# ikt-luh/Unified-Point-Cloud-Compression

Hardware: AMD Instinct MI355X
Metric: points/sec encode+decode, longdress vox10, 1 GPU; bpp & D1-PSNR parity (higher is better)
Workload: dtype f32

## Files before the change

unified_point_cloud_compression_amd/csrc/pcc_conv_thin.hip:

```cpp
#include "pcc_conv.h"

struct ThinArgs {
  const float* feat; const float* wt; const float* bias;
  const int* hdr; const int* nbr; const int* rows;
  float* out; long long n_out; int cin, cout, act; float slope; int lpr_log2;
};

template <int COUT_MAX, int VEC>
__global__ void __launch_bounds__(256) k_conv_thin(ThinArgs a) {
  typedef typename ThinVec<VEC>::T VT;
  constexpr int JB = 9;
  const int lane = threadIdx.x & 63;
  const int lpr = 1 << a.lpr_log2;
  const int rpw = 64 >> a.lpr_log2;
  const long long wave = (long long)blockIdx.x * 4 + (threadIdx.x >> 6);
  const long long p = wave * rpw + (lane >> a.lpr_log2);
  const int cl = lane & (lpr - 1);
  const bool valid = p < a.n_out;
  const int cvec = a.cin / VEC;

  int k_count = 1, koff_begin = 0;
  long long seg_pos_count = a.n_out, local = p;
  const int* seg_nbr = nullptr;
  const bool identity = (a.hdr == nullptr);
  if (!identity && valid) {
    const int nseg = a.hdr[HDR_NSEG];
    int s = 0;
    for (; s < nseg - 1; ++s) {
      const int* sg = a.hdr + HDR_SEG0 + s * SEG_WORDS;
      if (p < (long long)sg[SEG_POS_BEGIN] + sg[SEG_POS_COUNT]) break;
    }
    const int* sg = a.hdr + HDR_SEG0 + s * SEG_WORDS;
    k_count = sg[SEG_K_COUNT];
    koff_begin = sg[SEG_KOFF_BEGIN];
    seg_pos_count = sg[SEG_POS_COUNT];
    local = p - sg[SEG_POS_BEGIN];
    seg_nbr = a.nbr + (((long long)(unsigned)sg[SEG_NBR_LO]) | ((long long)sg[SEG_NBR_HI] << 32));
  }
  float acc[COUT_MAX];
#pragma unroll
  for (int o = 0; o < COUT_MAX; ++o) acc[o] = 0.f;
  if (valid) {
    for (int cv = cl; cv < cvec; cv += lpr) {
      for (int j0 = 0; j0 < k_count; j0 += JB) {
        int ir[JB];
#pragma unroll
        for (int u = 0; u < JB; ++u) {
          const int j = j0 + u;
          ir[u] = (j < k_count) ? (identity ? (int)p : seg_nbr[(long long)j * seg_pos_count + local]) : -1;
        }
        VT x[JB];
#pragma unroll
        for (int u = 0; u < JB; ++u) {
          thin_zero(x[u]);
          if (ir[u] >= 0) x[u] = reinterpret_cast<const VT*>(a.feat + (long long)ir[u] * a.cin)[cv];
        }
#pragma unroll
        for (int u = 0; u < JB; ++u) {
          const int j = j0 + u;
          if (j < k_count) {
            const int kid = identity ? 0 : a.hdr[HDR_KOFFS + koff_begin + j];
            const float* wk = a.wt + (long long)kid * a.cout * a.cin;
#pragma unroll
            for (int o = 0; o < COUT_MAX; ++o)
              if (o < a.cout) acc[o] += thin_dot(x[u], reinterpret_cast<const VT*>(wk + o * a.cin)[cv]);
          }
        }
      }
    }
  }
#pragma unroll
  for (int o = 0; o < COUT_MAX; ++o)
    for (int d = lpr >> 1; d >= 1; d >>= 1) acc[o] += __shfl_xor(acc[o], d);
  if (valid && cl == 0) {
    const long long orow = a.rows ? a.rows[p] : p;
#pragma unroll
    for (int o = 0; o < COUT_MAX; ++o) {
      if (o >= a.cout) break;
      float v = acc[o] + (a.bias ? a.bias[o] : 0.f);
      if (a.act == PCC_ACT_RELU) v = fmaxf(v, 0.f);
      else if (a.act == PCC_ACT_LEAKY) v = v >= 0.f ? v : v * a.slope;
      a.out[orow * a.cout + o] = v;
    }
  }
}

template <int CIN>
__global__ void __launch_bounds__(256) k_thin_project(const float* __restrict__ feat, long long n_in,
                                                      const float* __restrict__ wt, int kc, float* __restrict__ t) {
  extern __shared__ __attribute__((aligned(16))) float w_s[];
  for (int i = threadIdx.x; i < kc * CIN; i += 256) w_s[i] = wt[i];
  __syncthreads();
  const long long i = (long long)blockIdx.x * 256 + threadIdx.x;
  if (i >= n_in) return;
  float4 x[CIN / 4];
#pragma unroll
  for (int c = 0; c < CIN / 4; ++c) x[c] = reinterpret_cast<const float4*>(feat + i * CIN)[c];
  for (int k = 0; k < kc; ++k) {
    float acc = 0.f;
#pragma unroll
    for (int c = 0; c < CIN / 4; ++c) {
      const float4 w = reinterpret_cast<const float4*>(w_s + k * CIN)[c];
      acc += x[c].x * w.x + x[c].y * w.y + x[c].z * w.z + x[c].w * w.w;
    }
    t[(long long)k * n_in + i] = acc;
  }
}

struct ThinGatherArgs {
  const float* t; const float* bias; const int* hdr; const int* nbr; const int* rows;
  float* out; long long n_in, n_out; int cout, act; float slope;
};

template <int COUT_MAX>
__global__ void __launch_bounds__(256) k_thin_gather(ThinGatherArgs a) {
  constexpr int JB = 9;
  const long long p = (long long)blockIdx.x * 256 + threadIdx.x;
  if (p >= a.n_out) return;
  int k_count = 1, koff_begin = 0;
  long long spc = a.n_out, local = p;
  const int* seg_nbr = nullptr;
  const bool identity = (a.hdr == nullptr);
  if (!identity) {
    const int nseg = a.hdr[HDR_NSEG];
    int s = 0;
    for (; s < nseg - 1; ++s) {
      const int* sg = a.hdr + HDR_SEG0 + s * SEG_WORDS;
      if (p < (long long)sg[SEG_POS_BEGIN] + sg[SEG_POS_COUNT]) break;
    }
    const int* sg = a.hdr + HDR_SEG0 + s * SEG_WORDS;
    k_count = sg[SEG_K_COUNT]; koff_begin = sg[SEG_KOFF_BEGIN]; spc = sg[SEG_POS_COUNT];
    local = p - sg[SEG_POS_BEGIN];
    seg_nbr = a.nbr + (((long long)(unsigned)sg[SEG_NBR_LO]) | ((long long)sg[SEG_NBR_HI] << 32));
  }
  float acc[COUT_MAX];
#pragma unroll
  for (int o = 0; o < COUT_MAX; ++o) acc[o] = 0.f;
  for (int j0 = 0; j0 < k_count; j0 += JB) {
    int ir[JB];
#pragma unroll
    for (int u = 0; u < JB; ++u)
      ir[u] = (j0 + u < k_count) ? (identity ? (int)p : seg_nbr[(long long)(j0 + u) * spc + local]) : -1;
    float v[JB][COUT_MAX];
#pragma unroll
    for (int u = 0; u < JB; ++u) {
      const int kid = (ir[u] >= 0 && !identity) ? a.hdr[HDR_KOFFS + koff_begin + j0 + u] : 0;
#pragma unroll
      for (int o = 0; o < COUT_MAX; ++o)
        v[u][o] = (ir[u] >= 0 && o < a.cout) ? a.t[(long long)(kid * a.cout + o) * a.n_in + ir[u]] : 0.f;
    }
#pragma unroll
    for (int u = 0; u < JB; ++u)
#pragma unroll
      for (int o = 0; o < COUT_MAX; ++o) acc[o] += v[u][o];
  }
  const long long orow = a.rows ? a.rows[p] : p;
#pragma unroll
  for (int o = 0; o < COUT_MAX; ++o)
    if (o < a.cout) a.out[orow * a.cout + o] = act1(acc[o] + (a.bias ? a.bias[o] : 0.f), a.act, a.slope);
}


struct Wave16Args {
  const float* feat; const float* wl; const float* bias; const int* hdr; const int* nbr; const int* rows;
  float* out; long long n_out, n_in; int K, cout, act; float slope;
  const int* tiles = nullptr; const int* n_tiles = nullptr;
  const float* w2 = nullptr;
  float* t = nullptr;
};

template <int CIN>
__device__ __forceinline__ const float* wave16_w(const float* wl_s, int kid, int kq, int r16) {
  return wl_s + ((kid * (CIN / 4) + kq) * 16 + r16) * 4;
}

template <int CIN>
__global__ void __launch_bounds__(512) k_conv_wave16(Wave16Args a) {
  constexpr int G = CIN / 16;
  constexpr int NW = 8;
  extern __shared__ __attribute__((aligned(16))) float wl_s[];
  for (int i = threadIdx.x; i < a.K * 16 * (CIN / 4); i += 512)
    reinterpret_cast<float4*>(wl_s)[i] = reinterpret_cast<const float4*>(a.wl)[i];
  __syncthreads();
  const int lane = threadIdx.x & 63, r16 = lane & 15, q = lane >> 4;
  const bool identity = (a.hdr == nullptr);
  const int nseg = identity ? 1 : a.hdr[HDR_NSEG];
  long long total_tiles = 0;
  if (identity) total_tiles = (a.n_out + 31) / 32;
  else
    for (int s = 0; s < nseg; ++s) total_tiles += (a.hdr[HDR_SEG0 + s * SEG_WORDS + SEG_POS_COUNT] + 31) / 32;

  const int cpx = gridDim.x >> 3;
  const long long per_xcd = (total_tiles + 7) / 8;
  const long long xcd_lo = (long long)(blockIdx.x & 7) * per_xcd;
  const long long xcd_hi = min(total_tiles, xcd_lo + per_xcd);
  for (long long wt = xcd_lo + (long long)(blockIdx.x >> 3) * NW + (threadIdx.x >> 6); wt < xcd_hi;
       wt += (long long)cpx * NW) {
    long long pos0, spc;
    int npos, k_count = 1, koff_begin = 0;
    const int* seg_nbr = nullptr;
    if (identity) {
      pos0 = wt * 32; npos = (int)min(32ll, a.n_out - pos0); spc = a.n_out;
    } else {
      long long tile = wt;
      int s = 0;
      for (; s < nseg - 1; ++s) {
        const long long tiles = (a.hdr[HDR_SEG0 + s * SEG_WORDS + SEG_POS_COUNT] + 31) / 32;
        if (tile < tiles) break;
        tile -= tiles;
      }
      const int* sg = a.hdr + HDR_SEG0 + s * SEG_WORDS;
      k_count = sg[SEG_K_COUNT]; koff_begin = sg[SEG_KOFF_BEGIN]; spc = sg[SEG_POS_COUNT];
      const long long local0 = tile * 32;
      pos0 = sg[SEG_POS_BEGIN] + local0;
      npos = (int)min(32ll, spc - local0);
      seg_nbr = a.nbr + (((long long)(unsigned)sg[SEG_NBR_LO]) | ((long long)sg[SEG_NBR_HI] << 32)) + local0;
    }
    const bool vA = r16 < npos, vB = 16 + r16 < npos;
    f32x4 accA0 = {0.f, 0.f, 0.f, 0.f}, accA1 = accA0, accB0 = accA0, accB1 = accA0;
    auto fetch = [&](int j, int& iA, int& iB) {
      iA = -1; iB = -1;
      if (j < k_count) {
        if (vA) iA = identity ? (int)(pos0 + r16) : seg_nbr[(long long)j * spc + r16];
        if (vB) iB = identity ? (int)(pos0 + 16 + r16) : seg_nbr[(long long)j * spc + 16 + r16];
      }
    };
    auto gather = [&](int iA, int iB, float4 (&xa)[G], float4 (&xb)[G]) {
#pragma unroll
      for (int g = 0; g < G; ++g) {
        xa[g] = make_float4(0.f, 0.f, 0.f, 0.f);
        xb[g] = xa[g];
        if (iA >= 0) xa[g] = *reinterpret_cast<const float4*>(a.feat + (long long)iA * CIN + 16 * g + 4 * q);
        if (iB >= 0) xb[g] = *reinterpret_cast<const float4*>(a.feat + (long long)iB * CIN + 16 * g + 4 * q);
      }
    };
    int iA0, iB0, iA1, iB1, iA2, iB2;
    float4 xa[G], xb[G], ya[G], yb[G];
    fetch(0, iA0, iB0);
    fetch(1, iA1, iB1);
    gather(iA0, iB0, xa, xb);
    for (int j = 0; j < k_count; ++j) {
      fetch(j + 2, iA2, iB2);
      gather(iA1, iB1, ya, yb);
      if (__ballot(iA0 >= 0 || iB0 >= 0)) {
        const int kid = identity ? 0 : a.hdr[HDR_KOFFS + koff_begin + j];
#pragma unroll
        for (int g = 0; g < G; ++g) {
          const float4 w = *reinterpret_cast<const float4*>(wave16_w<CIN>(wl_s, kid, 4 * g + q, r16));
          accA0 = __builtin_amdgcn_mfma_f32_16x16x4f32(xa[g].x, w.x, accA0, 0, 0, 0);
          accB0 = __builtin_amdgcn_mfma_f32_16x16x4f32(xb[g].x, w.x, accB0, 0, 0, 0);
          accA1 = __builtin_amdgcn_mfma_f32_16x16x4f32(xa[g].y, w.y, accA1, 0, 0, 0);
          accB1 = __builtin_amdgcn_mfma_f32_16x16x4f32(xb[g].y, w.y, accB1, 0, 0, 0);
          accA0 = __builtin_amdgcn_mfma_f32_16x16x4f32(xa[g].z, w.z, accA0, 0, 0, 0);
          accB0 = __builtin_amdgcn_mfma_f32_16x16x4f32(xb[g].z, w.z, accB0, 0, 0, 0);
          accA1 = __builtin_amdgcn_mfma_f32_16x16x4f32(xa[g].w, w.w, accA1, 0, 0, 0);
          accB1 = __builtin_amdgcn_mfma_f32_16x16x4f32(xb[g].w, w.w, accB1, 0, 0, 0);
        }
      }
#pragma unroll
      for (int g = 0; g < G; ++g) { xa[g] = ya[g]; xb[g] = yb[g]; }
      iA0 = iA1; iB0 = iB1; iA1 = iA2; iB1 = iB2;
    }
    if (r16 < a.cout) {
      const float b = a.bias ? a.bias[r16] : 0.f;
#pragma unroll
      for (int e = 0; e < 4; ++e) {
        const int rA = 4 * q + e, rB = 16 + 4 * q + e;
        if (rA < npos) {
          const long long orow = a.rows ? a.rows[pos0 + rA] : pos0 + rA;
          a.out[orow * a.cout + r16] = act1(accA0[e] + accA1[e] + b, a.act, a.slope);
        }
        if (rB < npos) {
          const long long orow = a.rows ? a.rows[pos0 + rB] : pos0 + rB;
          a.out[orow * a.cout + r16] = act1(accB0[e] + accB1[e] + b, a.act, a.slope);
        }
      }
    }
  }
}

template <int CTRL>
__device__ __forceinline__ int dpp_i(int v) { return __builtin_amdgcn_update_dpp(0, v, CTRL, 0xF, 0xF, true); }
template <int CTRL>
__device__ __forceinline__ float dpp_f(float v) {
  return __builtin_bit_cast(float, __builtin_amdgcn_update_dpp(0, __builtin_bit_cast(int, v), CTRL, 0xF, 0xF, true));
}
static constexpr int DPP_SHL1 = 0x101, DPP_SHR1 = 0x111;

template <int CIN, bool PROJ>
__global__ void __launch_bounds__(512) k_conv_wave16z(Wave16Args a) {
  constexpr int G = CIN / 16;
  constexpr int NW = 8;
  extern __shared__ __attribute__((aligned(16))) float wl_s[];
  for (int i = threadIdx.x; i < 27 * 16 * (CIN / 4); i += 512)
    reinterpret_cast<float4*>(wl_s)[i] = reinterpret_cast<const float4*>(a.wl)[i];
  __syncthreads();
  const int lane = threadIdx.x & 63, r16 = lane & 15, q = lane >> 4;
  const unsigned spc = (unsigned)a.n_out;
  const unsigned total_tiles = a.tiles ? (unsigned)*a.n_tiles : (spc + 15) / 16;
  const unsigned cpx = gridDim.x >> 3;
  const unsigned per_xcd = (total_tiles + 7) / 8;
  const unsigned xcd_lo = (blockIdx.x & 7) * per_xcd;
  const unsigned xcd_hi = min(total_tiles, xcd_lo + per_xcd);
  const float* wl_lane = wl_s + r16 * 4 + q * 64;

  float w2r[2][4];
  float* hs = nullptr;
  if constexpr (PROJ) {
#pragma unroll
    for (int nt = 0; nt < 2; ++nt)
#pragma unroll
      for (int j = 0; j < 4; ++j) {
        const int k = 16 * nt + r16, c = 4 * j + q;
        w2r[nt][j] = (k < 27 && c < a.cout) ? a.w2[k * a.cout + c] : 0.f;
      }
    hs = wl_s + 27 * 16 * CIN + (threadIdx.x >> 6) * (16 * 17);
  }

  struct Grp { float4 c[G], m[G], p[G]; unsigned km, kp; };
  const __amdgpu_buffer_rsrc_t rs = __builtin_amdgcn_make_buffer_rsrc(
      const_cast<float*>(a.feat), (short)0, (int)(unsigned)((size_t)a.n_in * CIN * 4), 0x00020000);
  constexpr unsigned OOB = 0xFFFFFF00u;

  for (unsigned wt = xcd_lo + (blockIdx.x >> 3) * NW + (threadIdx.x >> 6); wt < xcd_hi; wt += cpx * NW) {
    unsigned pos0, npos;
    if (a.tiles) {
      const unsigned tw = (unsigned)a.tiles[wt];
      pos0 = tw & 0x07FFFFFFu; npos = (tw >> 27) + 1;
    } else {
      pos0 = wt * 16; npos = min(16u, spc - pos0);
    }
    const unsigned r = pos0 + min((unsigned)r16, npos - 1);
    const int* nb = a.nbr + r;
    f32x4 acc0 = {0.f, 0.f, 0.f, 0.f}, acc1 = acc0, acc2 = acc0, acc3 = acc0;

    auto issue = [&](int im, int ic, int ip, Grp& x) {
      const int cm = dpp_i<DPP_SHR1>(ic), cp = dpp_i<DPP_SHL1>(ic);
      const bool mm = im >= 0 && im == cm && r16 != 0;
      const bool mp = ip >= 0 && ip == cp && r16 != 15;
      x.km = mm ? 0xFFFFFFFFu : 0u;
      x.kp = mp ? 0xFFFFFFFFu : 0u;
      asm volatile("" : "+v"(x.km), "+v"(x.kp));
      const unsigned oc = ic >= 0 ? (unsigned)ic * (CIN * 4) + 16 * q : OOB;
      const unsigned om = (im >= 0 && !mm) ? (unsigned)im * (CIN * 4) + 16 * q : OOB;
      const unsigned op = (ip >= 0 && !mp) ? (unsigned)ip * (CIN * 4) + 16 * q : OOB;
#pragma unroll
      for (int g = 0; g < G; ++g) {
        x.c[g] = __builtin_bit_cast(float4, __builtin_amdgcn_raw_buffer_load_b128(rs, oc + 64 * g, 0, 0));
        x.m[g] = __builtin_bit_cast(float4, __builtin_amdgcn_raw_buffer_load_b128(rs, om + 64 * g, 0, 0));
        x.p[g] = __builtin_bit_cast(float4, __builtin_amdgcn_raw_buffer_load_b128(rs, op + 64 * g, 0, 0));
      }
    };
    auto mfma4 = [&](const float4& x, int slot, int g) {
      const float4 w = *reinterpret_cast<const float4*>(wl_lane + (slot * (CIN / 4) + 4 * g) * 64);
      acc0 = __builtin_amdgcn_mfma_f32_16x16x4f32(x.x, w.x, acc0, 0, 0, 0);
      acc1 = __builtin_amdgcn_mfma_f32_16x16x4f32(x.y, w.y, acc1, 0, 0, 0);
      acc2 = __builtin_amdgcn_mfma_f32_16x16x4f32(x.z, w.z, acc2, 0, 0, 0);
      acc3 = __builtin_amdgcn_mfma_f32_16x16x4f32(x.w, w.w, acc3, 0, 0, 0);
    };
    auto mix = [](unsigned k, float shifted, float loaded) {
      return __builtin_bit_cast(float, (__builtin_bit_cast(unsigned, shifted) & k) | __builtin_bit_cast(unsigned, loaded));
    };

    int im1 = nb[spc], ic1 = nb[10ull * spc], ip1 = nb[19ull * spc];
    Grp x, y;
    issue(nb[0], nb[9ull * spc], nb[18ull * spc], x);
    auto compute = [&](const Grp& x, int g9) {
#pragma unroll
      for (int g = 0; g < G; ++g) {
        float4 vm, vp;
        vm.x = mix(x.km, dpp_f<DPP_SHR1>(x.c[g].x), x.m[g].x);  vp.x = mix(x.kp, dpp_f<DPP_SHL1>(x.c[g].x), x.p[g].x);
        vm.y = mix(x.km, dpp_f<DPP_SHR1>(x.c[g].y), x.m[g].y);  vp.y = mix(x.kp, dpp_f<DPP_SHL1>(x.c[g].y), x.p[g].y);
        vm.z = mix(x.km, dpp_f<DPP_SHR1>(x.c[g].z), x.m[g].z);  vp.z = mix(x.kp, dpp_f<DPP_SHL1>(x.c[g].z), x.p[g].z);
        vm.w = mix(x.km, dpp_f<DPP_SHR1>(x.c[g].w), x.m[g].w);  vp.w = mix(x.kp, dpp_f<DPP_SHL1>(x.c[g].w), x.p[g].w);
        mfma4(vm, g9, g);
        mfma4(x.c[g], g9 + 9, g);
        mfma4(vp, g9 + 18, g);
      }
    };
#pragma unroll 1
    for (int g9 = 0; g9 < 8; g9 += 2) {
      const unsigned ga = (unsigned)(g9 + 2), gb = (unsigned)min(g9 + 3, 8);
      const int am = nb[(size_t)ga * spc], ac = nb[(size_t)(ga + 9) * spc], ap = nb[(size_t)(ga + 18) * spc];
      issue(im1, ic1, ip1, y);
      __builtin_amdgcn_sched_barrier(0);
      compute(x, g9);
      __builtin_amdgcn_sched_barrier(0);
      const int bm = nb[(size_t)gb * spc], bc = nb[(size_t)(gb + 9) * spc], bp = nb[(size_t)(gb + 18) * spc];
      issue(am, ac, ap, x);
      __builtin_amdgcn_sched_barrier(0);
      compute(y, g9 + 1);
      __builtin_amdgcn_sched_barrier(0);
      im1 = bm; ic1 = bc; ip1 = bp;
    }
    compute(x, 8);
    const float b = (a.bias && r16 < a.cout) ? a.bias[r16] : 0.f;
    if constexpr (!PROJ) {
      if (r16 < a.cout) {
#pragma unroll
        for (int e = 0; e < 4; ++e) {
          const unsigned lr = 4 * q + e;
          if (lr < npos) a.out[(size_t)(pos0 + lr) * a.cout + r16] = act1(acc0[e] + acc1[e] + acc2[e] + acc3[e] + b, a.act, a.slope);
        }
      }
    } else {
#pragma unroll
      for (int e = 0; e < 4; ++e)
        hs[(4 * q + e) * 17 + r16] = r16 < a.cout ? act1(acc0[e] + acc1[e] + acc2[e] + acc3[e] + b, a.act, a.slope) : 0.f;
      __builtin_amdgcn_wave_barrier();
      f32x4 d0 = {0.f, 0.f, 0.f, 0.f}, d1 = d0;
#pragma unroll
      for (int j = 0; j < 4; ++j) {
        const float hv = hs[r16 * 17 + 4 * j + q];
        d0 = __builtin_amdgcn_mfma_f32_16x16x4f32(w2r[0][j], hv, d0, 0, 0, 0);
        d1 = __builtin_amdgcn_mfma_f32_16x16x4f32(w2r[1][j], hv, d1, 0, 0, 0);
      }
      __builtin_amdgcn_wave_barrier();
      if ((unsigned)r16 < npos) {
        float* tp = a.t + (size_t)(4 * q) * spc + pos0 + r16;
#pragma unroll
        for (int e = 0; e < 4; ++e) {
          tp[(size_t)e * spc] = d0[e];
          if (16 + 4 * q + e < 27) tp[(size_t)(16 + e) * spc] = d1[e];
        }
      }
    }
  }
}

static bool g_wave16_zrun = getenv("PCC_WAVE16_ZRUN") ? atoi(getenv("PCC_WAVE16_ZRUN")) != 0 : true;

template <int CIN>
static int launch_wave16(const Wave16Args& a, hipStream_t s) {
  const size_t lds = (size_t)a.K * 16 * CIN * sizeof(float);
  int dev = 0;
  PCC_CHECK_HIP(hipGetDevice(&dev));
  static unsigned long long attr_set = 0;
  if (!(attr_set >> (dev & 63) & 1ull)) {
    PCC_CHECK_HIP(hipFuncSetAttribute((const void*)k_conv_wave16<CIN>, hipFuncAttributeMaxDynamicSharedMemorySize, 64 * 1024));
    PCC_CHECK_HIP(hipFuncSetAttribute((const void*)k_conv_wave16z<CIN, false>, hipFuncAttributeMaxDynamicSharedMemorySize, 64 * 1024));
    PCC_CHECK_HIP(hipFuncSetAttribute((const void*)k_conv_wave16z<CIN, true>, hipFuncAttributeMaxDynamicSharedMemorySize, 64 * 1024));
    attr_set |= 1ull << (dev & 63);
  }
  prof_note(PCC_FORM_WAVE16, 0.0, 0.0);
  prof_tile(32, 16, 1);
  const long long tiles = pcc_cdiv(a.n_out, 32) + (a.rows ? PCC_MAP_MAX_SEG : 0);
  long long want = pcc_cdiv(tiles, 8);
  want = (want + 7) / 8 * 8;
  const unsigned grid = (unsigned)(want < 512 ? want : 512);
  if (g_wave16_zrun && a.K == 27 && a.hdr && !a.rows && a.n_out * 27 < (1ll << 31) &&
      a.n_in * CIN * 4 <= 0xFFFFFE00ll) {
    if (a.t) k_conv_wave16z<CIN, true><<<grid, 512, lds + 8 * 16 * 17 * sizeof(float), s>>>(a);
    else k_conv_wave16z<CIN, false><<<grid, 512, lds, s>>>(a);
    PCC_LAUNCH_CHECK();
    return PCC_OK;
  }
  PCC_REQUIRE(!a.t, "pcc_conv_head_fwd: the fused head needs a canonical 3x3x3 map (one segment, no row list)");
  k_conv_wave16<CIN><<<grid, 512, lds, s>>>(a);
  PCC_LAUNCH_CHECK();
  return PCC_OK;
}

template <int CIN>
__global__ void __launch_bounds__(256) k_thin_project_mfma(const float* __restrict__ feat, long long n_in,
                                                           const float* __restrict__ wt, int kc, float* __restrict__ t) {
  constexpr int HC = CIN / 2, NV = HC / 4;
  const int lane = threadIdx.x & 63, r31 = lane & 31, half = lane >> 5;
  const long long ntiles = (n_in + 31) / 32;
  float wa[HC];
#pragma unroll
  for (int c = 0; c < HC; ++c) wa[c] = r31 < kc ? wt[r31 * CIN + half * HC + c] : 0.f;
  const long long tstep = (long long)gridDim.x * 4;
  long long tile = (long long)blockIdx.x * 4 + (threadIdx.x >> 6);
  if (tile >= ntiles) return;
  auto load = [&](long long tl, float4 (&x)[NV]) {
    long long row = tl * 32 + r31;
    if (row >= n_in) row = n_in - 1;
    const float4* src = reinterpret_cast<const float4*>(feat + row * CIN + half * HC);
#pragma unroll
    for (int v = 0; v < NV; ++v) x[v] = src[v];
  };
  auto run = [&](long long tl, const float4 (&x)[NV]) {
    f32x16 acc;
#pragma unroll
    for (int e = 0; e < 16; ++e) acc[e] = 0.f;
#pragma unroll
    for (int v = 0; v < NV; ++v) {
      acc = __builtin_amdgcn_mfma_f32_32x32x2f32(wa[4 * v + 0], x[v].x, acc, 0, 0, 0);
      acc = __builtin_amdgcn_mfma_f32_32x32x2f32(wa[4 * v + 1], x[v].y, acc, 0, 0, 0);
      acc = __builtin_amdgcn_mfma_f32_32x32x2f32(wa[4 * v + 2], x[v].z, acc, 0, 0, 0);
      acc = __builtin_amdgcn_mfma_f32_32x32x2f32(wa[4 * v + 3], x[v].w, acc, 0, 0, 0);
    }
    const long long row = tl * 32 + r31;
    if (row < n_in) {
#pragma unroll
      for (int e = 0; e < 16; ++e) {
        const int k = cfrag_row(0, e, half);
        if (k < kc) t[(long long)k * n_in + row] = acc[e];
      }
    }
  };
  float4 xa[NV], xb[NV];
  load(tile, xa);
  for (;;) {
    const long long t1 = tile + tstep;
    if (t1 < ntiles) load(t1, xb);
    run(tile, xa);
    if (t1 >= ntiles) break;
    const long long t2 = t1 + tstep;
    if (t2 < ntiles) load(t2, xa);
    run(t1, xb);
    if (t2 >= ntiles) break;
    tile = t2;
  }
}

template <int CIN>
static int launch_project(const float* feat, int64_t n_in, const float* wt, int kc, float* t, hipStream_t s) {
  if constexpr (CIN >= 32) {
    if (kc <= 32) {
      const long long tiles = pcc_cdiv(n_in, 32);
      long long grid = pcc_cdiv(tiles, 4 * 4);
      if (grid > 4096) grid = 4096;
      if (grid < 1) grid = 1;
      k_thin_project_mfma<CIN><<<(unsigned)grid, 256, 0, s>>>(feat, n_in, wt, kc, t);
      PCC_LAUNCH_CHECK();
      return PCC_OK;
    }
  }
  k_thin_project<CIN><<<(unsigned)pcc_cdiv(n_in, 256), 256, (size_t)kc * CIN * sizeof(float), s>>>(feat, n_in, wt, kc, t);
  PCC_LAUNCH_CHECK();
  return PCC_OK;
}

int launch_conv_wave16(const float* feat_in, int64_t n_in, int32_t cin, const float* packed_w, const float* bias, int32_t K,
                       int32_t cout, const int32_t* hdr, const int32_t* nbr, const int32_t* rows, int64_t n_out, float* out,
                       int32_t act, float slope, hipStream_t s, const int32_t* tiles, const int32_t* n_tiles, const float* w2,
                       float* t) {
  Wave16Args a;
  a.feat = feat_in; a.wl = packed_w; a.bias = bias; a.hdr = hdr; a.nbr = nbr; a.rows = rows; a.out = out;
  a.n_out = n_out; a.n_in = n_in; a.K = K; a.cout = cout; a.act = act; a.slope = slope;
  a.tiles = tiles; a.n_tiles = n_tiles; a.w2 = w2; a.t = t;
  if (cin == 16) PCC_TRY(launch_wave16<16>(a, s));
  else if (cin == 32) PCC_TRY(launch_wave16<32>(a, s));
  else PCC_TRY(launch_wave16<64>(a, s));
  return PCC_OK;
}

int launch_conv_thin_t(const float* feat_in, int64_t n_in, int32_t cin, const float* packed_w, const float* bias, int32_t K,
                       int32_t cout, const int32_t* hdr, const int32_t* nbr, const int32_t* rows, int64_t n_out, float* out,
                       int32_t act, float slope, void* ws, size_t ws_bytes, hipStream_t s) {
  if (!ws || ws_bytes < pcc_conv_ws_bytes(n_in, K, cin, cout)) {
    pcc_set_error("pcc_conv_fwd: workspace too small (need pcc_conv_ws_bytes)");
    return PCC_EWS;
  }
  float* t = (float*)ws;
  const int kc = K * cout;
  switch (cin) {
    case 4: PCC_TRY(launch_project<4>(feat_in, n_in, packed_w, kc, t, s)); break;
    case 8: PCC_TRY(launch_project<8>(feat_in, n_in, packed_w, kc, t, s)); break;
    case 16: PCC_TRY(launch_project<16>(feat_in, n_in, packed_w, kc, t, s)); break;
    case 32: PCC_TRY(launch_project<32>(feat_in, n_in, packed_w, kc, t, s)); break;
    default: PCC_TRY(launch_project<64>(feat_in, n_in, packed_w, kc, t, s)); break;
  }
  ThinGatherArgs g;
  g.t = t; g.bias = bias; g.hdr = hdr; g.nbr = nbr; g.rows = rows; g.out = out; g.n_in = n_in; g.n_out = n_out;
  g.cout = cout; g.act = act; g.slope = slope;
  k_thin_gather<4><<<(unsigned)pcc_cdiv(n_out, 256), 256, 0, s>>>(g);
  PCC_LAUNCH_CHECK();
  return PCC_OK;
}

int launch_conv_thin(const float* feat_in, int32_t cin, const float* packed_w, const float* bias, int32_t cout, const int32_t* hdr,
                     const int32_t* nbr, const int32_t* rows, int64_t n_out, float* out, int32_t act, float slope, hipStream_t s) {
  ThinArgs t;
  t.feat = feat_in; t.wt = packed_w; t.bias = bias; t.hdr = hdr; t.nbr = nbr; t.rows = rows; t.out = out;
  t.n_out = n_out; t.cin = cin; t.cout = cout; t.act = act; t.slope = slope;
  const int vec = (cin % 4 == 0) ? 4 : 1;
  int l = 0;
  while ((1 << l) < cin / vec && l < 6) ++l;
  t.lpr_log2 = l;
  const int64_t rpw = 64 >> l;
  const int64_t waves = pcc_cdiv(n_out, rpw);
  if (vec == 4) k_conv_thin<4, 4><<<(unsigned)pcc_cdiv(waves, 4), 256, 0, s>>>(t);
  else k_conv_thin<4, 1><<<(unsigned)pcc_cdiv(waves, 4), 256, 0, s>>>(t);
  PCC_LAUNCH_CHECK();
  return PCC_OK;
}

__global__ void k_band_segments(const long long* __restrict__ keys, long long n, int lo_x, int nx, int lo_y, int ny, int ts,
                                int nbands, int band_h, int* __restrict__ seg_row0, int* __restrict__ seg_tiles) {
  const int sidx = blockIdx.x * blockDim.x + threadIdx.x;
  if (sidx >= nbands * nx) return;
  const int band = sidx / nx, xi = sidx - band * nx;
  const long long x = (long long)lo_x + (long long)xi * ts + PCC_BIAS;
  const int cy0 = band * band_h, cy1 = min(ny, cy0 + band_h);
  auto lower = [&](long long key) {
    long long lo = 0, hi = n;
    while (lo < hi) {
      const long long mid = (lo + hi) >> 1;
      if (keys[mid] < key) lo = mid + 1; else hi = mid;
    }
    return lo;
  };
  long long b = 0, e = 0;
  if (cy0 < cy1) {
    const long long y0 = (long long)lo_y + (long long)cy0 * ts + PCC_BIAS, y1 = (long long)lo_y + (long long)cy1 * ts + PCC_BIAS;
    b = lower((x << PCC_KEY_X_SHIFT) | (y0 << PCC_KEY_Y_SHIFT));
    e = lower((x << PCC_KEY_X_SHIFT) | (y1 << PCC_KEY_Y_SHIFT));
  }
  seg_row0[sidx] = (int)b;
  seg_tiles[sidx] = (int)((e - b + 15) / 16);
  seg_row0[nbands * nx + sidx] = (int)(e - b);
}

__global__ void __launch_bounds__(1024) k_band_scan(const int* __restrict__ seg_tiles, int nseg, int* __restrict__ seg_tile0,
                                                    int* __restrict__ n_tiles) {
  __shared__ int part[1024];
  const int per = (nseg + 1023) / 1024;
  const int b = threadIdx.x * per, e = min(nseg, b + per);
  int sum = 0;
  for (int i = b; i < e; ++i) sum += seg_tiles[i];
  part[threadIdx.x] = sum;
  __syncthreads();
  for (int d = 1; d < 1024; d <<= 1) {
    const int v = threadIdx.x >= d ? part[threadIdx.x - d] : 0;
    __syncthreads();
    part[threadIdx.x] += v;
    __syncthreads();
  }
  int run = part[threadIdx.x] - sum;
  for (int i = b; i < e; ++i) { seg_tile0[i] = run; run += seg_tiles[i]; }
  if (threadIdx.x == 1023) *n_tiles = part[1023];
}

__global__ void __launch_bounds__(256) k_band_fill(const int* __restrict__ seg_row0, const int* __restrict__ seg_rows,
                                                   const int* __restrict__ seg_tile0, int nseg, int* __restrict__ tiles) {
  const int sidx = blockIdx.x * 4 + (threadIdx.x >> 6);
  if (sidx >= nseg) return;
  const int rows = seg_rows[sidx], r0 = seg_row0[sidx], t0 = seg_tile0[sidx];
  const int nt = (rows + 15) / 16;
  for (int j = threadIdx.x & 63; j < nt; j += 64) {
    const int cnt = min(16, rows - 16 * j);
    tiles[t0 + j] = (r0 + 16 * j) | ((cnt - 1) << 27);
  }
}

extern "C" int64_t pcc_band_tiles_cap(int64_t n, int32_t nx, int32_t nbands) { return n / 16 + (int64_t)nx * nbands + 16; }
extern "C" size_t pcc_band_tiles_ws_bytes(int32_t nx, int32_t nbands) { return pcc_align_up((size_t)nx * nbands * 4) * 4 + 256; }

extern "C" int pcc_band_tiles_build(const int64_t* keys, int64_t n, int32_t lo_x, int32_t nx, int32_t lo_y, int32_t ny,
                                    int32_t ts, int32_t nbands, int32_t* tiles, int64_t tiles_cap, int32_t* n_tiles,
                                    void* ws, size_t ws_bytes, void* stream) {
  hipStream_t s = (hipStream_t)stream;
  PCC_REQUIRE(keys && tiles && n_tiles && ws && n > 0 && n < (1ll << 27), "pcc_band_tiles_build: bad arguments (rows must stay below 2^27)");
  PCC_REQUIRE(nx >= 1 && ny >= 1 && ts >= 1 && nbands >= 1 && (int64_t)nx * nbands <= (1 << 20), "pcc_band_tiles_build: bad lattice");
  PCC_REQUIRE(tiles_cap >= pcc_band_tiles_cap(n, nx, nbands), "pcc_band_tiles_build: tile table too small (pcc_band_tiles_cap)");
  if (ws_bytes < pcc_band_tiles_ws_bytes(nx, nbands)) { pcc_set_error("pcc_band_tiles_build: workspace too small"); return PCC_EWS; }
  const int nseg = nx * nbands;
  const size_t st = pcc_align_up((size_t)nseg * 4);
  int* seg_row0 = (int*)ws;
  int* seg_tiles = (int*)((char*)ws + 2 * st);
  int* seg_tile0 = (int*)((char*)ws + 3 * st);
  PCC_REQUIRE(st >= (size_t)nseg * 4, "pcc_band_tiles_build: internal");
  const int band_h = (ny + nbands - 1) / nbands;
  k_band_segments<<<(unsigned)pcc_cdiv(nseg, 256), 256, 0, s>>>((const long long*)keys, n, lo_x, nx, lo_y, ny, ts, nbands, band_h,
                                                                seg_row0, seg_tiles);
  PCC_LAUNCH_CHECK();
  k_band_scan<<<1, 1024, 0, s>>>(seg_tiles, nseg, seg_tile0, n_tiles);
  PCC_LAUNCH_CHECK();
  k_band_fill<<<(unsigned)pcc_cdiv(nseg, 4), 256, 0, s>>>(seg_row0, seg_row0 + nseg, seg_tile0, nseg, tiles);
  PCC_LAUNCH_CHECK();
  return PCC_OK;
}

extern "C" int pcc_conv_head_supported(int32_t cin, int32_t cmid) {
  return (cmid > 4 && cmid <= 16 && conv_kind(27, cin, cmid) == KIND_WAVE16 && (size_t)27 * 16 * cin * 4 + 8 * 16 * 17 * 4 <= 64 * 1024) ? 1 : 0;
}
extern "C" size_t pcc_conv_head_ws_bytes(int64_t n) { return (size_t)27 * (size_t)(n > 0 ? n : 1) * sizeof(float) + 256; }

extern "C" int pcc_conv_head_fwd(const float* feat, int64_t n, int32_t cin, const float* packed_w0, const float* bias0,
                                 int32_t cmid, const float* w2, const float* bias2, const int32_t* hdr, const int32_t* nbr,
                                 const int32_t* tiles, const int32_t* n_tiles, float* logits, void* ws, size_t ws_bytes,
                                 void* stream) {
  hipStream_t s = (hipStream_t)stream;
  if (n <= 0) return PCC_OK;
  PCC_REQUIRE(feat && packed_w0 && w2 && hdr && nbr && logits && ws, "pcc_conv_head_fwd: NULL array");
  PCC_REQUIRE(pcc_conv_head_supported(cin, cmid), "pcc_conv_head_fwd: unsupported shape cin=%d cmid=%d", cin, cmid);
  PCC_REQUIRE((tiles == nullptr) == (n_tiles == nullptr), "pcc_conv_head_fwd: tiles and n_tiles go together");
  PCC_REQUIRE(n * 27 < (1ll << 31) && n * cin * 4 <= 0xFFFFFE00ll && g_wave16_zrun, "pcc_conv_head_fwd: set too large for 32-bit offsets");
  if (ws_bytes < pcc_conv_head_ws_bytes(n)) { pcc_set_error("pcc_conv_head_fwd: workspace too small"); return PCC_EWS; }
  PCC_TRY(prof_begin(s));
  PCC_TRY(launch_conv_wave16(feat, n, cin, packed_w0, bias0, 27, cmid, hdr, nbr, nullptr, n, nullptr, PCC_ACT_RELU, 0.f, s, tiles,
                             n_tiles, w2, (float*)ws));
  PCC_TRY(prof_end(s));
  ThinGatherArgs g;
  g.t = (const float*)ws; g.bias = bias2; g.hdr = hdr; g.nbr = nbr; g.rows = nullptr; g.out = logits; g.n_in = n; g.n_out = n;
  g.cout = 1; g.act = PCC_ACT_NONE; g.slope = 0.f;
  k_thin_gather<1><<<(unsigned)pcc_cdiv(n, 256), 256, 0, s>>>(g);
  PCC_LAUNCH_CHECK();
  return PCC_OK;
}

struct ThinGridArgs {
  const float* t; const float* bias; const long long* keys; PccGrid g; float* out; long long n; int cout;
};

template <int COUT_MAX>
__global__ void __launch_bounds__(256) k_thin_gather_grid(ThinGridArgs a) {
  const long long p = (long long)blockIdx.x * 256 + threadIdx.x;
  if (p >= a.n) return;
  const PccGrid& g = a.g;
  const long long key = a.keys[p];
  const PccLattice& L = g.lat;
  const int b = pcc_key_b(key);
  const int cx = (pcc_key_x(key) - L.lo[0]) >> L.ts_log2;
  const int cy = (pcc_key_y(key) - L.lo[1]) >> L.ts_log2;
  const int cz = (pcc_key_z(key) - L.lo[2]) >> L.ts_log2;
  const int z_lo = cz > 0 ? cz - 1 : 0, z_hi = cz + 1 < L.dims[2] ? cz + 1 : L.dims[2] - 1;
  const int nz = z_hi - z_lo + 1;
  float acc[COUT_MAX];
#pragma unroll
  for (int o = 0; o < COUT_MAX; ++o) acc[o] = 0.f;
#pragma unroll
  for (int c = 0; c < 9; ++c) {
    const int nx = cx + c % 3 - 1, ny = cy + c / 3 - 1;
    if (nx < 0 || ny < 0 || nx >= L.dims[0] || ny >= L.dims[1]) continue;
    const long long cell = (((long long)b * L.dims[0] + nx) * L.dims[1] + ny) * L.dims[2] + z_lo;
    const long long wi = cell >> 6;
    const int sh = (int)(cell & 63);
    const unsigned long long w0 = g.bits[wi];
    unsigned long long f64 = w0 >> sh;
    if (sh + nz > 64) f64 |= g.bits[wi + 1] << (64 - sh);
    unsigned f = (unsigned)f64 & ((1u << nz) - 1u);
    if (!f) continue;
    int r = g.rank[wi] + __popcll(w0 & ((1ull << sh) - 1ull));
    while (f) {
      const int t = __ffs((int)f) - 1;
      f &= f - 1;
      const int k = c + 9 * (z_lo + t - cz + 1);
#pragma unroll
      for (int o = 0; o < COUT_MAX; ++o)
        if (o < a.cout) acc[o] += a.t[(long long)(k * a.cout + o) * a.n + r];
      ++r;
    }
  }
#pragma unroll
  for (int o = 0; o < COUT_MAX; ++o)
    if (o < a.cout) a.out[p * a.cout + o] = acc[o] + (a.bias ? a.bias[o] : 0.f);
}

__global__ void __launch_bounds__(256) k_thin_gather_grid1(ThinGridArgs a) {
  const long long p = (long long)blockIdx.x * 256 + threadIdx.x;
  if (p >= a.n) return;
  const PccGrid& g = a.g;
  const long long key = a.keys[p];
  const PccLattice& L = g.lat;
  const int b = pcc_key_b(key);
  const int cx = (pcc_key_x(key) - L.lo[0]) >> L.ts_log2;
  const int cy = (pcc_key_y(key) - L.lo[1]) >> L.ts_log2;
  const int cz = (pcc_key_z(key) - L.lo[2]) >> L.ts_log2;
  const int z_lo = cz > 0 ? cz - 1 : 0, z_hi = cz + 1 < L.dims[2] ? cz + 1 : L.dims[2] - 1;
  const int nz = z_hi - z_lo + 1;
  const int dz0 = z_lo - cz + 1;
  unsigned long long w0[9], w1[9];
  int rk[9], sh[9];
  bool ok[9];
#pragma unroll
  for (int c = 0; c < 9; ++c) {
    const int nx = cx + c % 3 - 1, ny = cy + c / 3 - 1;
    ok[c] = !(nx < 0 || ny < 0 || nx >= L.dims[0] || ny >= L.dims[1]);
    const long long cell = ok[c] ? pcc_lat_cell(L, b, nx, ny, z_lo) : 0ll;
    const long long wi = cell >> 6;
    sh[c] = (int)(cell & 63);
    w0[c] = g.bits[wi];
    rk[c] = g.rank[wi];
    w1[c] = (sh[c] + nz > 64) ? g.bits[wi + 1] : 0ull;
  }
  const __amdgpu_buffer_rsrc_t rsT = __builtin_amdgcn_make_buffer_rsrc(const_cast<float*>(a.t), (short)0,
                                                                       (int)(unsigned)((size_t)27 * a.n * 4), 0x00020000);
  float v[27];
#pragma unroll
  for (int c = 0; c < 9; ++c) {
    unsigned long long f64 = w0[c] >> sh[c];
    if (sh[c] + nz > 64) f64 |= w1[c] << (64 - sh[c]);
    const unsigned f = ok[c] ? ((unsigned)f64 & ((1u << nz) - 1u)) : 0u;
    const int r = rk[c] + __popcll(w0[c] & ((1ull << sh[c]) - 1ull));
#pragma unroll
    for (int t = 0; t < 3; ++t) {
      const int k = c + 9 * (dz0 + t);
      const unsigned row = (unsigned)(r + __popc(f & ((1u << t) - 1u)));
      const unsigned off = ((f >> t) & 1u) ? ((unsigned)k * (unsigned)a.n + row) * 4u : BUF_OOB;
      v[c * 3 + t] = __builtin_bit_cast(float, __builtin_amdgcn_raw_buffer_load_b32(rsT, off, 0, 0));
    }
  }
  float acc = 0.f;
#pragma unroll
  for (int i = 0; i < 27; ++i) acc += v[i];
  a.out[p] = acc + (a.bias ? a.bias[0] : 0.f);
}

template <int CIN>
__global__ void __launch_bounds__(256) k_thin_project_z(const float* __restrict__ feat, const long long* __restrict__ keys,
                                                        long long n_in, long long ts, const float* __restrict__ wt,
                                                        float* __restrict__ t) {
  extern __shared__ __attribute__((aligned(16))) float w_s[];
  __shared__ float sd[27][258];
  for (int i = threadIdx.x; i < 27 * CIN; i += 256) w_s[i] = wt[i];
  __syncthreads();
  const long long base = (long long)blockIdx.x * 256;
  const long long i = base + threadIdx.x;
  const bool valid = i < n_in;
  float4 x[CIN / 4];
#pragma unroll
  for (int c = 0; c < CIN / 4; ++c) x[c] = valid ? reinterpret_cast<const float4*>(feat + i * CIN)[c] : make_float4(0.f, 0.f, 0.f, 0.f);
  const long long key = valid ? keys[i] : -(1ll << 62);
  const bool adjm = valid && i > 0 && keys[i - 1] == key - ts;
  const bool adjp = valid && i + 1 < n_in && keys[i + 1] == key + ts;
#pragma unroll 1
  for (int k = 0; k < 27; ++k) {
    float acc = 0.f;
#pragma unroll
    for (int c = 0; c < CIN / 4; ++c) {
      const float4 w = reinterpret_cast<const float4*>(w_s + k * CIN)[c];
      acc += x[c].x * w.x + x[c].y * w.y + x[c].z * w.z + x[c].w * w.w;
    }
    sd[k][1 + threadIdx.x] = acc;
  }
  if (threadIdx.x < 18) {
    const int e = threadIdx.x < 9 ? threadIdx.x : threadIdx.x - 9;
    const long long r = threadIdx.x < 9 ? base - 1 : base + 256;
    const int k = threadIdx.x < 9 ? e : e + 18;
    float acc = 0.f;
    if (r >= 0 && r < n_in) {
#pragma unroll
      for (int c = 0; c < CIN / 4; ++c) {
        const float4 xv = reinterpret_cast<const float4*>(feat + r * CIN)[c];
        const float4 w = reinterpret_cast<const float4*>(w_s + k * CIN)[c];
        acc += xv.x * w.x + xv.y * w.y + xv.z * w.z + xv.w * w.w;
      }
    }
    sd[k][threadIdx.x < 9 ? 0 : 257] = acc;
  }
  __syncthreads();
  if (!valid) return;
  const int col = 1 + threadIdx.x;
#pragma unroll 1
  for (int g = 0; g < 9; ++g) {
    const float lo = sd[g][col], mid = sd[g + 9][col], hi = sd[g + 18][col];
    const float from_dn = sd[g][col - 1];
    const float from_up = sd[g + 18][col + 1];
    t[(long long)g * n_in + i] = (mid + (adjm ? from_dn : 0.f)) + (adjp ? from_up : 0.f);
    t[(long long)(9 + g) * n_in + i] = lo;
    t[(long long)(18 + g) * n_in + i] = hi;
  }
}

__global__ void __launch_bounds__(256) k_thin_gather_grid1z(ThinGridArgs a) {
  const long long p = (long long)blockIdx.x * 256 + threadIdx.x;
  if (p >= a.n) return;
  const PccGrid& g = a.g;
  const long long key = a.keys[p];
  const PccLattice& L = g.lat;
  const int b = pcc_key_b(key);
  const int cx = (pcc_key_x(key) - L.lo[0]) >> L.ts_log2;
  const int cy = (pcc_key_y(key) - L.lo[1]) >> L.ts_log2;
  const int cz = (pcc_key_z(key) - L.lo[2]) >> L.ts_log2;
  const int z_lo = cz > 0 ? cz - 1 : 0, z_hi = cz + 1 < L.dims[2] ? cz + 1 : L.dims[2] - 1;
  const int nz = z_hi - z_lo + 1;
  const int dz0 = z_lo - cz + 1;
  unsigned long long w0[9], w1[9];
  int rk[9], sh[9];
  bool ok[9];
#pragma unroll
  for (int c = 0; c < 9; ++c) {
    const int nx = cx + c % 3 - 1, ny = cy + c / 3 - 1;
    ok[c] = !(nx < 0 || ny < 0 || nx >= L.dims[0] || ny >= L.dims[1]);
    const long long cell = ok[c] ? pcc_lat_cell(L, b, nx, ny, z_lo) : 0ll;
    const long long wi = cell >> 6;
    sh[c] = (int)(cell & 63);
    w0[c] = g.bits[wi];
    rk[c] = g.rank[wi];
    w1[c] = (sh[c] + nz > 64) ? g.bits[wi + 1] : 0ull;
  }
  const __amdgpu_buffer_rsrc_t rsT = __builtin_amdgcn_make_buffer_rsrc(const_cast<float*>(a.t), (short)0,
                                                                       (int)(unsigned)((size_t)27 * a.n * 4), 0x00020000);
  const int tm = 1 - dz0;
  float v[27];
#pragma unroll
  for (int c = 0; c < 9; ++c) {
    unsigned long long f64 = w0[c] >> sh[c];
    if (sh[c] + nz > 64) f64 |= w1[c] << (64 - sh[c]);
    const unsigned f = ok[c] ? ((unsigned)f64 & ((1u << nz) - 1u)) : 0u;
    const unsigned r = (unsigned)(rk[c] + __popcll(w0[c] & ((1ull << sh[c]) - 1ull)));
    const bool mid = (f >> tm) & 1u;
    const bool low = dz0 == 0 && (f & 1u);
    const int tu = 2 - dz0;
    const bool upp = tu < nz && ((f >> tu) & 1u);
    const unsigned row_mid = r + __popc(f & ((1u << tm) - 1u));
    const unsigned row_up = r + __popc(f & ((1u << tu) - 1u));
    const unsigned n = (unsigned)a.n;
    const unsigned o_s = mid ? ((unsigned)c * n + row_mid) * 4u : BUF_OOB;
    const unsigned o_u = (!mid && low) ? ((unsigned)(9 + c) * n + r) * 4u : BUF_OOB;
    const unsigned o_d = (!mid && upp) ? ((unsigned)(18 + c) * n + row_up) * 4u : BUF_OOB;
    v[c * 3 + 0] = __builtin_bit_cast(float, __builtin_amdgcn_raw_buffer_load_b32(rsT, o_s, 0, 0));
    v[c * 3 + 1] = __builtin_bit_cast(float, __builtin_amdgcn_raw_buffer_load_b32(rsT, o_u, 0, 0));
    v[c * 3 + 2] = __builtin_bit_cast(float, __builtin_amdgcn_raw_buffer_load_b32(rsT, o_d, 0, 0));
  }
  float acc = 0.f;
#pragma unroll
  for (int i = 0; i < 27; ++i) acc += v[i];
  a.out[p] = acc + (a.bias ? a.bias[0] : 0.f);
}

static long long g_thin_z_min_rows = 1ll << 20;
extern "C" int pcc_set_thin_z_min_rows(int64_t rows) { g_thin_z_min_rows = rows; return PCC_OK; }

extern "C" size_t pcc_thin_grid_ws_bytes(int64_t n, int32_t cout) { return (size_t)27 * cout * (size_t)(n > 0 ? n : 1) * sizeof(float) + 256; }

extern "C" int pcc_conv_thin_grid_fwd(const float* feat, int64_t n, int32_t cin, const float* packed_w ,
                                      const float* bias, int32_t cout, const int64_t* keys, const uint64_t* bits,
                                      const int32_t* rank, const int32_t* h_grid, float* out, void* ws, size_t ws_bytes,
                                      void* stream) {
  hipStream_t s = (hipStream_t)stream;
  if (n <= 0) return PCC_OK;
  PCC_REQUIRE(feat && packed_w && keys && bits && rank && out && ws, "pcc_conv_thin_grid_fwd: NULL array");
  PccGrid g;
  PCC_TRY(pcc_grid_from_host(bits, rank, h_grid, "pcc_conv_thin_grid_fwd", &g));
  PCC_REQUIRE(cout >= 1 && cout <= 4 && conv_kind(27, cin, cout) == KIND_THIN_T, "pcc_conv_thin_grid_fwd: unsupported shape cin=%d cout=%d", cin, cout);
  if (ws_bytes < pcc_thin_grid_ws_bytes(n, cout)) { pcc_set_error("pcc_conv_thin_grid_fwd: workspace too small"); return PCC_EWS; }
  float* t = (float*)ws;
  const int kc = 27 * cout;
  if (g_thin_z_min_rows >= 0 && cout == 1 && cin == 16 && (size_t)27 * n * 4 <= (size_t)BUF_MAX_BYTES && n >= g_thin_z_min_rows) {
    k_thin_project_z<16><<<(unsigned)pcc_cdiv(n, 256), 256, (size_t)27 * 16 * sizeof(float), s>>>(
        feat, (const long long*)keys, n, (long long)h_grid[6], packed_w, t);
    ThinGridArgs az;
    az.t = t; az.bias = bias; az.keys = (const long long*)keys; az.g = g; az.out = out; az.n = n; az.cout = 1;
    k_thin_gather_grid1z<<<(unsigned)pcc_cdiv(n, 256), 256, 0, s>>>(az);
    PCC_LAUNCH_CHECK();
    return PCC_OK;
  }
  switch (cin) {
    case 4: PCC_TRY(launch_project<4>(feat, n, packed_w, kc, t, s)); break;
    case 8: PCC_TRY(launch_project<8>(feat, n, packed_w, kc, t, s)); break;
    case 16: PCC_TRY(launch_project<16>(feat, n, packed_w, kc, t, s)); break;
    case 32: PCC_TRY(launch_project<32>(feat, n, packed_w, kc, t, s)); break;
    default: PCC_TRY(launch_project<64>(feat, n, packed_w, kc, t, s)); break;
  }
  ThinGridArgs a;
  a.t = t; a.bias = bias; a.keys = (const long long*)keys; a.g = g; a.out = out; a.n = n; a.cout = cout;
  if (cout == 1 && (size_t)27 * n * 4 <= (size_t)BUF_MAX_BYTES) k_thin_gather_grid1<<<(unsigned)pcc_cdiv(n, 256), 256, 0, s>>>(a);
  else if (cout == 1) k_thin_gather_grid<1><<<(unsigned)pcc_cdiv(n, 256), 256, 0, s>>>(a);
  else k_thin_gather_grid<4><<<(unsigned)pcc_cdiv(n, 256), 256, 0, s>>>(a);
  PCC_LAUNCH_CHECK();
  return PCC_OK;
}
```

Before: 54.20 million.

## Recompute sparse z-boundary projections in gather instead of storing lo/hi planes

The z-fused thin projection now writes only the 9 merged planes instead of 27. The gather kernel compacts the rare lo/hi boundary requests per wave with ballot/mbcnt into shared memory, and recomputes those dot products directly from the features and weights. Weights are read straight from global memory rather than staged through shared memory. This removes two thirds of the projection's write and read traffic, at the cost of 16KB of shared memory per block, extra wave-level bookkeeping, and a 26-bit row limit.

```diff
diff --git a/unified_point_cloud_compression_amd/csrc/pcc_conv_thin.hip b/unified_point_cloud_compression_amd/csrc/pcc_conv_thin.hip
--- a/unified_point_cloud_compression_amd/csrc/pcc_conv_thin.hip
+++ b/unified_point_cloud_compression_amd/csrc/pcc_conv_thin.hip
@@ -800,14 +800,34 @@
   a.out[p] = acc + (a.bias ? a.bias[0] : 0.f);
 }
 
+
+template <int CIN>
+__device__ __forceinline__ float thin_z_dot(const float4 (&x)[CIN / 4], const float4 (&w)[CIN / 4]) {
+  float acc = 0.f;
+#pragma unroll
+  for (int c = 0; c < CIN / 4; ++c) {
+    float g = x[c].y * w[c].y;
+    g = __builtin_fmaf(x[c].x, w[c].x, g);
+    g = __builtin_fmaf(x[c].z, w[c].z, g);
+    g = __builtin_fmaf(x[c].w, w[c].w, g);
+    acc += g;
+  }
+  return acc;
+}
+template <int CIN>
+__device__ __forceinline__ float thin_z_dot_unfused(const float4 (&x)[CIN / 4], const float4 (&w)[CIN / 4]) {
+#pragma clang fp contract(off)
+  float acc = 0.f;
+#pragma unroll
+  for (int c = 0; c < CIN / 4; ++c) acc += x[c].x * w[c].x + x[c].y * w[c].y + x[c].z * w[c].z + x[c].w * w[c].w;
+  return acc;
+}
+
 template <int CIN>
 __global__ void __launch_bounds__(256) k_thin_project_z(const float* __restrict__ feat, const long long* __restrict__ keys,
                                                         long long n_in, long long ts, const float* __restrict__ wt,
                                                         float* __restrict__ t) {
-  extern __shared__ __attribute__((aligned(16))) float w_s[];
   __shared__ float sd[27][258];
-  for (int i = threadIdx.x; i < 27 * CIN; i += 256) w_s[i] = wt[i];
-  __syncthreads();
   const long long base = (long long)blockIdx.x * 256;
   const long long i = base + threadIdx.x;
   const bool valid = i < n_in;
@@ -817,15 +837,12 @@
   const long long key = valid ? keys[i] : -(1ll << 62);
   const bool adjm = valid && i > 0 && keys[i - 1] == key - ts;
   const bool adjp = valid && i + 1 < n_in && keys[i + 1] == key + ts;
-#pragma unroll 1
+#pragma unroll 3
   for (int k = 0; k < 27; ++k) {
-    float acc = 0.f;
-#pragma unroll
-    for (int c = 0; c < CIN / 4; ++c) {
-      const float4 w = reinterpret_cast<const float4*>(w_s + k * CIN)[c];
-      acc += x[c].x * w.x + x[c].y * w.y + x[c].z * w.z + x[c].w * w.w;
-    }
-    sd[k][1 + threadIdx.x] = acc;
+    float4 w[CIN / 4];
+#pragma unroll
+    for (int c = 0; c < CIN / 4; ++c) w[c] = reinterpret_cast<const float4*>(wt + k * CIN)[c];
+    sd[k][1 + threadIdx.x] = thin_z_dot<CIN>(x, w);
   }
   if (threadIdx.x < 18) {
     const int e = threadIdx.x < 9 ? threadIdx.x : threadIdx.x - 9;
@@ -833,12 +850,13 @@
     const int k = threadIdx.x < 9 ? e : e + 18;
     float acc = 0.f;
     if (r >= 0 && r < n_in) {
+      float4 xv[CIN / 4], w[CIN / 4];
 #pragma unroll
       for (int c = 0; c < CIN / 4; ++c) {
-        const float4 xv = reinterpret_cast<const float4*>(feat + r * CIN)[c];
-        const float4 w = reinterpret_cast<const float4*>(w_s + k * CIN)[c];
-        acc += xv.x * w.x + xv.y * w.y + xv.z * w.z + xv.w * w.w;
-      }
+        xv[c] = reinterpret_cast<const float4*>(feat + r * CIN)[c];
+        w[c] = reinterpret_cast<const float4*>(wt + k * CIN)[c];
+      }
+      acc = thin_z_dot_unfused<CIN>(xv, w);
     }
     sd[k][threadIdx.x < 9 ? 0 : 257] = acc;
   }
@@ -847,20 +865,26 @@
   const int col = 1 + threadIdx.x;
 #pragma unroll 1
   for (int g = 0; g < 9; ++g) {
-    const float lo = sd[g][col], mid = sd[g + 9][col], hi = sd[g + 18][col];
+    const float mid = sd[g + 9][col];
     const float from_dn = sd[g][col - 1];
     const float from_up = sd[g + 18][col + 1];
     t[(long long)g * n_in + i] = (mid + (adjm ? from_dn : 0.f)) + (adjp ? from_up : 0.f);
-    t[(long long)(9 + g) * n_in + i] = lo;
-    t[(long long)(18 + g) * n_in + i] = hi;
-  }
-}
-
-__global__ void __launch_bounds__(256) k_thin_gather_grid1z(ThinGridArgs a) {
+  }
+}
+
+struct ThinGridZArgs : ThinGridArgs {
+  const float* feat; const float* wt;
+};
+static constexpr int THIN_Z_ITEMS = 16 * 64;
+
+__global__ void __launch_bounds__(256) k_thin_gather_grid1z(ThinGridZArgs a) {
+  __shared__ unsigned item_s[4][THIN_Z_ITEMS];
   const long long p = (long long)blockIdx.x * 256 + threadIdx.x;
-  if (p >= a.n) return;
+  const bool valid = p < a.n;
+  const int lane = threadIdx.x & 63;
+  unsigned* const items = item_s[threadIdx.x >> 6];
   const PccGrid& g = a.g;
-  const long long key = a.keys[p];
+  const long long key = valid ? a.keys[p] : 0ll;
   const PccLattice& L = g.lat;
   const int b = pcc_key_b(key);
   const int cx = (pcc_key_x(key) - L.lo[0]) >> L.ts_log2;
@@ -875,7 +899,7 @@
 #pragma unroll
   for (int c = 0; c < 9; ++c) {
     const int nx = cx + c % 3 - 1, ny = cy + c / 3 - 1;
-    ok[c] = !(nx < 0 || ny < 0 || nx >= L.dims[0] || ny >= L.dims[1]);
+    ok[c] = valid && !(nx < 0 || ny < 0 || nx >= L.dims[0] || ny >= L.dims[1]);
     const long long cell = ok[c] ? pcc_lat_cell(L, b, nx, ny, z_lo) : 0ll;
     const long long wi = cell >> 6;
     sh[c] = (int)(cell & 63);
@@ -884,9 +908,12 @@
     w1[c] = (sh[c] + nz > 64) ? g.bits[wi + 1] : 0ull;
   }
   const __amdgpu_buffer_rsrc_t rsT = __builtin_amdgcn_make_buffer_rsrc(const_cast<float*>(a.t), (short)0,
-                                                                       (int)(unsigned)((size_t)27 * a.n * 4), 0x00020000);
+                                                                       (int)(unsigned)((size_t)9 * a.n * 4), 0x00020000);
   const int tm = 1 - dz0;
   float v[27];
+  int pos[18];
+  unsigned wants = 0u;
+  int cnt = 0;
 #pragma unroll
   for (int c = 0; c < 9; ++c) {
     unsigned long long f64 = w0[c] >> sh[c];
@@ -899,18 +926,42 @@
     const bool upp = tu < nz && ((f >> tu) & 1u);
     const unsigned row_mid = r + __popc(f & ((1u << tm) - 1u));
     const unsigned row_up = r + __popc(f & ((1u << tu) - 1u));
-    const unsigned n = (unsigned)a.n;
-    const unsigned o_s = mid ? ((unsigned)c * n + row_mid) * 4u : BUF_OOB;
-    const unsigned o_u = (!mid && low) ? ((unsigned)(9 + c) * n + r) * 4u : BUF_OOB;
-    const unsigned o_d = (!mid && upp) ? ((unsigned)(18 + c) * n + row_up) * 4u : BUF_OOB;
-    v[c * 3 + 0] = __builtin_bit_cast(float, __builtin_amdgcn_raw_buffer_load_b32(rsT, o_s, 0, 0));
-    v[c * 3 + 1] = __builtin_bit_cast(float, __builtin_amdgcn_raw_buffer_load_b32(rsT, o_u, 0, 0));
-    v[c * 3 + 2] = __builtin_bit_cast(float, __builtin_amdgcn_raw_buffer_load_b32(rsT, o_d, 0, 0));
-  }
+    const unsigned o_s = mid ? ((unsigned)c * (unsigned)a.n + row_mid) * 4u : BUF_OOB;
+    v[c * 3] = __builtin_bit_cast(float, __builtin_amdgcn_raw_buffer_load_b32(rsT, o_s, 0, 0));
+#pragma unroll
+    for (int u = 0; u < 2; ++u) {
+      const bool want = !mid && (u ? upp : low);
+      wants |= want ? 1u << (2 * c + u) : 0u;
+      const unsigned long long bal = __ballot(want);
+      const int at = cnt + (int)__builtin_amdgcn_mbcnt_hi((unsigned)(bal >> 32), __builtin_amdgcn_mbcnt_lo((unsigned)bal, 0u));
+      pos[2 * c + u] = want ? at : 0;
+      if (want) items[at] = (u ? row_up : r) | (unsigned)(2 * c + u) << 26;
+      cnt += (int)__popcll(bal);
+    }
+  }
+  const __amdgpu_buffer_rsrc_t rsH = __builtin_amdgcn_make_buffer_rsrc(const_cast<float*>(a.feat), (short)0,
+                                                                       (int)(unsigned)((size_t)a.n * 64), 0x00020000);
+  __builtin_amdgcn_wave_barrier();
+  for (int j = lane; j < cnt; j += 64) {
+    const unsigned it = items[j];
+    const unsigned row = it & 0x03FFFFFFu, slot = it >> 26;
+    const unsigned k = (slot >> 1) + ((slot & 1u) ? 18u : 0u);
+    float4 x[4], w[4];
+#pragma unroll
+    for (int c = 0; c < 4; ++c) {
+      x[c] = __builtin_bit_cast(float4, __builtin_amdgcn_raw_buffer_load_b128(rsH, row * 64u + c * 16u, 0, 0));
+      w[c] = reinterpret_cast<const float4*>(a.wt + k * 16u)[c];
+    }
+    items[j] = __builtin_bit_cast(unsigned, thin_z_dot<16>(x, w));
+  }
+  __builtin_amdgcn_wave_barrier();
+#pragma unroll
+  for (int s = 0; s < 18; ++s)
+    v[(s >> 1) * 3 + 1 + (s & 1)] = ((wants >> s) & 1u) ? __builtin_bit_cast(float, items[pos[s]]) : 0.f;
   float acc = 0.f;
 #pragma unroll
   for (int i = 0; i < 27; ++i) acc += v[i];
-  a.out[p] = acc + (a.bias ? a.bias[0] : 0.f);
+  if (valid) a.out[p] = acc + (a.bias ? a.bias[0] : 0.f);
 }
 
 static long long g_thin_z_min_rows = 1ll << 20;
@@ -932,10 +983,11 @@
   float* t = (float*)ws;
   const int kc = 27 * cout;
   if (g_thin_z_min_rows >= 0 && cout == 1 && cin == 16 && (size_t)27 * n * 4 <= (size_t)BUF_MAX_BYTES && n >= g_thin_z_min_rows) {
-    k_thin_project_z<16><<<(unsigned)pcc_cdiv(n, 256), 256, (size_t)27 * 16 * sizeof(float), s>>>(
+    k_thin_project_z<16><<<(unsigned)pcc_cdiv(n, 256), 256, 0, s>>>(
         feat, (const long long*)keys, n, (long long)h_grid[6], packed_w, t);
-    ThinGridArgs az;
+    ThinGridZArgs az;
     az.t = t; az.bias = bias; az.keys = (const long long*)keys; az.g = g; az.out = out; az.n = n; az.cout = 1;
+    az.feat = feat; az.wt = packed_w;
     k_thin_gather_grid1z<<<(unsigned)pcc_cdiv(n, 256), 256, 0, s>>>(az);
     PCC_LAUNCH_CHECK();
     return PCC_OK;
```

Measured after the change: 54.90 million, median of 6. +1.3%, better.
